# riveSunder/therldaisyworld

Hardware: AMD Instinct MI355X
Metric: cell-updates/sec (grid x batch), fused stencil+growth step (higher is better)
Workload: dtype f32

## Files before the change

therldaisyworld_amd/csrc/dw_api.hip:

```cpp
#include <hip/hip_runtime.h>

#include <cmath>
#include <cstdarg>
#include <cstdio>
#include <cstdlib>
#include <cstring>
#include <memory>
#include <new>
#include <type_traits>
#include <vector>

#include "../../include/daisyworld_hip.h"
#include "dw_kernels.hpp"
#include "dw_host_util.hpp"

using namespace dw;

static thread_local char g_err[512] = "";

static int fail(int code, const char* fmt, ...) {
    va_list ap;
    va_start(ap, fmt);
    vsnprintf(g_err, sizeof(g_err), fmt, ap);
    va_end(ap);
    return code;
}

#define HIPCHK(expr)                                                                           \
    do {                                                                                       \
        hipError_t e_ = (expr);                                                                \
        if (e_ != hipSuccess)                                                                  \
            return fail(e_ == hipErrorOutOfMemory ? DW_ENOMEM : DW_EHIP, "%s failed: %s (%s:%d)", \
                        #expr, hipGetErrorString(e_), __FILE__, __LINE__);                      \
    } while (0)

#define NEED(cond, code, ...)                      \
    do {                                           \
        if (!(cond)) return fail(code, __VA_ARGS__); \
    } while (0)

enum UnqKind { UNQ_F64 = 1, UNQ_F32 = 2 };
enum UnqOwner { OWN_NONE = 0, OWN_CUR = 1, OWN_PREV = 2 };

struct Switches {
    bool no_sym = false, no_pack = false, no_fuse = false, no_ring = false, no_episode_kernel = false,
         no_episode_wave = false, no_agent_fuse = false, no_agent_preapply = false, first_f64 = false,
         first_generic = false, force_rescan = false, test_hooks = false;
    int pack_min_strips = -1, strip_rows = 0, tile_rpt = 0, queue_cap = -1, mismatch_cap = -1;
    double first_slack = -1.0;
    char kernel[16] = {0};
    char text[256] = {0};
};
static const char* test_hook(const char* name) {
    return std::getenv("DW_TEST_HOOKS") ? std::getenv(name) : nullptr;
}
static Switches read_switches() {
    Switches w;
    auto note = [&](const char* name, const char* val) {
        const size_t n = std::strlen(w.text);
        snprintf(w.text + n, sizeof(w.text) - n, "%s%s%s%s", n ? " " : "", name, val ? "=" : "", val ? val : "");
    };
    auto flag = [&](const char* name, bool& dst) { if (std::getenv(name)) { dst = true; note(name, nullptr); } };
    auto num = [&](const char* name, int& dst, bool test) {
        if (const char* e = test ? test_hook(name) : std::getenv(name)) { dst = std::atoi(e); note(name, e); }
    };
    w.test_hooks = std::getenv("DW_TEST_HOOKS") != nullptr;
    flag("DW_NO_SYM", w.no_sym); flag("DW_NO_PACK", w.no_pack); flag("DW_NO_FUSE", w.no_fuse); flag("DW_NO_RING", w.no_ring);
    flag("DW_NO_EPISODE_KERNEL", w.no_episode_kernel); flag("DW_NO_EPISODE_WAVE", w.no_episode_wave);
    flag("DW_NO_AGENT_FUSE", w.no_agent_fuse); flag("DW_NO_AGENT_PREAPPLY", w.no_agent_preapply);
    flag("DW_FIRST_STEP_F64", w.first_f64); flag("DW_FIRST_GENERIC", w.first_generic);
    num("DW_PACK_MIN_STRIPS", w.pack_min_strips, false); num("DW_STRIP_ROWS", w.strip_rows, false);
    num("DW_TILE_RPT", w.tile_rpt, false);
    num("DW_TEST_QUEUE_CAP", w.queue_cap, true); num("DW_TEST_MISMATCH_CAP", w.mismatch_cap, true);
    if (test_hook("DW_TEST_FORCE_RESCAN")) { w.force_rescan = true; note("DW_TEST_FORCE_RESCAN", nullptr); }
    if (const char* e = test_hook("DW_TEST_FIRST_SLACK")) { w.first_slack = std::atof(e); note("DW_TEST_FIRST_SLACK", e); }
    if (const char* e = std::getenv("DW_KERNEL")) { snprintf(w.kernel, sizeof(w.kernel), "%s", e); note("DW_KERNEL", e); }
    return w;
}

enum StepKind { STEP_GENERIC, STEP_TILED, STEP_STREAM };
struct StepPlan {
    StepKind kind = STEP_GENERIC;
    int halo = 0;
    bool packed = false;
    bool allow_fuse = false;
    int fused_mode = kFusedOvl;
    bool sym_albedo = false;
    int tcq = 0, rpt = 0;
    Geom geom{};
    size_t tile_lds = 0;
    StripGeom sgeom{};
    FusedGeom fgeom{};
    int first_prec = 2;
    bool first_stream = false;
    FirstGeom first_geom{};
    bool need_fixq = false;
};

static thread_local int t_fail_in = 0;
struct DeviceMem {
    static int alloc(void** p, size_t n) {
        if (t_fail_in > 0 && --t_fail_in == 0) return hipErrorOutOfMemory;
        return hipMalloc(p, n);
    }
    static int release(void* p) { return hipFree(p); }
};
struct PinnedMem {
    static int alloc(void** p, size_t n) { return hipHostMalloc(p, n, hipHostMallocDefault); }
    static int release(void* p) { return hipHostFree(p); }
};
template <class T> using DevBuf = Buf<T, DeviceMem>;
template <class T> using PinnedBuf = Buf<T, PinnedMem>;

struct dw_handle {
    dw_params prm;
    hipStream_t stream = nullptr;
    bool own_stream = false;
    size_t cells = 0;
    DevBuf<plane_t> L16[2];
    DevBuf<plane_t> D16[2];
    int cur = 0;
    DevBuf<double> L64;
    DevBuf<double> D64;
    DevBuf<float> U32L;
    DevBuf<float> U32D;
    UnqKind unq_kind = UNQ_F64;
    UnqOwner unq = OWN_NONE;
    bool have_state = false;
    bool stepped = false;
    double L_last = 0.0;
    DevBuf<int> idx;
    DevBuf<double> st;
    DevBuf<int> action;
    DevBuf<int> action_tmp;
    bool have_agents = false;
    DevBuf<StatsDev> stats2[2];
    size_t stats_bytes = 0;
    int sp = 0;
    DevBuf<uint4> fixq;
    unsigned int qcap = 0;
    DevBuf<int> redo_tiles;
    Switches sw{};
    StepPlan plan{};
    DevBuf<int> done_at;
    DevBuf<int> agents_done_at;
// ... 315 lines not shown
static int halo_form(int W) { return W < 256 ? 3 : (W == 256 ? 0 : (W % 256 == 0 ? 1 : 2)); }

static int strip_rows(long groups, int H, long target) {
    int sr = 64;
    while (sr > 8 && groups * ((H + sr - 1) / sr) < target) sr >>= 1;
    return H < sr ? H : sr;
}

static StepPlan plan_steps(const dw_params& p, const Switches& sw) {
    StepPlan s;
    s.sym_albedo = (p.albedo_dark - p.albedo_bare) == -(p.albedo_light - p.albedo_bare) && !sw.no_sym;
    s.halo = halo_form(p.width);
    const int lpw = p.width / 4, wpr = lpw ? 64 / lpw : 0;
    const bool pack_shape = p.width >= 8 && p.width < 256 && wpr >= 1 && wpr * lpw * 10 >= 64 * 7 && !sw.no_pack;
    const long pack_strips = pack_shape ? (long)((p.batch + wpr - 1) / wpr) * ((p.height + 63) / 64) : 0;
    const bool packable = pack_shape && pack_strips >= (sw.pack_min_strips >= 0 ? sw.pack_min_strips : 512);
    const bool quads = p.precision != DW_PRECISION_F64 && p.width % 4 == 0;
    if (quads && (p.width >= 256 || packable) && std::strcmp(sw.kernel, "tiled") != 0) {
        s.kind = STEP_STREAM;
        s.packed = p.width < 256;
        StripGeom& g = s.sgeom;
        g.B = p.batch; g.H = p.height; g.W = p.width;
        g.ncs = (p.width + 255) / 256;
        g.lpw = s.packed ? lpw : 64;
        g.wpr = s.packed ? wpr : 1;
        const long groups = s.packed ? (p.batch + wpr - 1) / wpr : p.batch;
        g.SR = sw.strip_rows >= 1 ? (p.height < sw.strip_rows ? p.height : sw.strip_rows)
                                  : strip_rows(groups * g.ncs, p.height, 2048);
        g.nrs = (p.height + g.SR - 1) / g.SR;
        g.nstrips = (int)(groups * g.nrs * g.ncs);
        g.nwg = (g.nstrips + 3) / 4;
        g.chunk = (g.nwg + 7) / 8;
        g.qcap = kWaveQueueCap;
        int mcap = kMismatchCap;
        if (sw.queue_cap >= 0 && sw.queue_cap < kWaveQueueCap) g.qcap = sw.queue_cap;
        if (sw.mismatch_cap >= 0 && sw.mismatch_cap < kMismatchCap) mcap = sw.mismatch_cap;
        g.force_rescan = sw.force_rescan ? 1 : 0;
        s.allow_fuse = !sw.no_fuse;
        const bool ring = p.width == 1024 && !sw.no_ring;
        s.fused_mode = p.width <= 256 ? kFusedRot : (ring ? kFusedRing : kFusedOvl);
        FusedGeom& f = s.fgeom;
        f.B = p.batch; f.H = p.height; f.W = p.width;
        f.SR = g.SR;
        f.nrs = g.nrs;
        f.lpw = g.lpw; f.wpr = g.wpr;
        f.cols_per_strip = p.width <= 256 ? 256 : (ring ? 1024 : 248);
        f.ncs = s.packed ? 1 : (p.width + f.cols_per_strip - 1) / f.cols_per_strip;
        f.nstrips = (int)(groups * f.nrs * f.ncs);
        f.nwg = ring ? f.nstrips : (f.nstrips + 3) / 4;
        f.chunk = (f.nwg + 7) / 8;
        f.qcap = g.qcap;
        f.mcap = mcap;
        f.sure_need = 9 * p.n_agents + 9 * mcap + 1;
    } else if (quads && p.width >= 64) {
        s.kind = STEP_TILED;
        const int Wq = p.width / 4;
        if (Wq >= 64) {
            s.tcq = 64; s.rpt = 4;
            if (sw.tile_rpt == 2 || sw.tile_rpt == 4 || sw.tile_rpt == 8) s.rpt = sw.tile_rpt;
        }
        else if (Wq >= 32) { s.tcq = 32; s.rpt = 4; }
        else { s.tcq = 16; s.rpt = 2; }
        const int TR = (256 / s.tcq) * s.rpt;
        Geom& g = s.geom;
        g.B = p.batch; g.H = p.height; g.W = p.width; g.Wq = Wq;
        g.tiles_r = (p.height + TR - 1) / TR;
        g.tiles_c = (Wq + s.tcq - 1) / s.tcq;
        g.ntiles = p.batch * g.tiles_r * g.tiles_c;
        g.chunk = (g.ntiles + 7) / 8;
        g.qcap = kMaxFix;
        if (sw.queue_cap >= 0 && sw.queue_cap < kMaxFix) g.qcap = sw.queue_cap;
        s.tile_lds = (size_t)2 * (TR + 2) * (s.tcq + 2) * 4 * sizeof(float);
    }
    s.need_fixq = p.precision == DW_PRECISION_EXACT && s.kind == STEP_TILED;
    s.first_prec = p.precision == DW_PRECISION_FAST ? 1 : (p.precision == DW_PRECISION_EXACT && !sw.first_f64 ? 3 : 2);
    s.first_stream = (p.width % 256 == 0 || s.kind == STEP_STREAM) && s.first_prec != 2 && !sw.first_generic;
    if (s.first_stream) {
        FirstGeom& fg = s.first_geom;
        fg.B = p.batch; fg.H = p.height; fg.W = p.width;
        fg.lpw = s.packed ? lpw : 64;
        fg.wpr = s.packed ? wpr : 1;
        fg.ncs = s.packed ? 1 : (p.width + 255) / 256;
        const long groups = s.packed ? (p.batch + fg.wpr - 1) / fg.wpr : p.batch;
        fg.SR = strip_rows(groups * fg.ncs, p.height, 4096);
        fg.nrs = (p.height + fg.SR - 1) / fg.SR;
        fg.nstrips = (int)(groups * fg.nrs * fg.ncs);
    }
    return s;
}

static int ensure_fixq(dw_handle* h, const StepPlan& plan) {
    if (!plan.need_fixq) return DW_OK;
    const dw_params& p = h->prm;
    size_t per_q = (h->cells / 64 + kNumQueues - 1) / kNumQueues;
    if (per_q < 2048) per_q = 2048;
    per_q = (per_q + 255) / 256 * 256;
    const size_t max_tiles = (size_t)p.batch * ((p.height + 7) / 8) * ((p.width / 4 + 15) / 16);
    if (int rc = alloc_group(h, "the near-tie queues", {{h->fixq, sizeof(uint4) * 3 * per_q * kNumQueues},
                                                         {h->redo_tiles, sizeof(int) * max_tiles}}))
        return rc;
    h->qcap = (unsigned int)per_q;
    return DW_OK;
}

struct StepOut {
    plane_t* L; plane_t* D;
// ... 87 lines not shown
        auto tiled = [&](auto TCQ, auto RPT) {
            return with_bool(ex, [&](auto EX) { return launch_tiled<TCQ, RPT, EX>(h, iL, iD, o, fq); });
        };
        if (pl.tcq == 64) return with_int<8, 4, 2>(pl.rpt, [&](auto RPT) { return tiled(int_c<64>{}, RPT); });
        return pl.tcq == 32 ? tiled(int_c<32>{}, int_c<4>{}) : tiled(int_c<16>{}, int_c<2>{});
    }
    HIPCHK(hipGetLastError());
    return DW_OK;
}

static void step_done(dw_handle* h, double L, bool stepped) {
    h->cur = 1 - h->cur;
    h->sp = 1 - h->sp;
    h->unq = h->unq == OWN_CUR ? OWN_PREV : OWN_NONE;
    h->stepped = stepped;
    h->L_last = L;
    release_unquantised(h);
}

static int launch_forward(dw_handle* h, double L) {
    const dw_params& p = h->prm;
    NEED(h->have_state, DW_ESTATE, "no state uploaded (call dw_upload_state_* or dw_init_random)");
    const int out = 1 - h->cur;
    StatsDev* stats = h->stats2[1 - h->sp].get();
    const StepOut o{h->L16[out].get(), h->D16[out].get(), derive_f32(p, L), make_f64(p, L), stats, &stats[p.batch].sum_l,
                    reinterpret_cast<unsigned long long*>(h->stats2[h->sp].get()),
                    (int)(h->stats_bytes / sizeof(unsigned long long))};
#ifdef DW_TUNING
    if (const char* e = std::getenv("DW_ABLATE")) {
        if (std::strcmp(e, "copy") == 0) {
            const int in = h->cur;
            const size_t n4 = h->cells * sizeof(plane_t) / 16;
            hipLaunchKernelGGL(copy_planes, dim3((unsigned)((n4 + 255) / 256)), dim3(256), 0, h->stream,
                               reinterpret_cast<const float4*>(h->L16[in].get()), reinterpret_cast<const float4*>(h->D16[in].get()),
                               reinterpret_cast<float4*>(h->L16[out].get()), reinterpret_cast<float4*>(h->D16[out].get()), n4);
            HIPCHK(hipGetLastError());
            h->cur = out; h->sp = 1 - h->sp; h->stepped = true; h->L_last = L;
            return DW_OK;
        }
        const int v = std::strcmp(e, "nomath") == 0 ? 1 : 0;
        HIPCHK(hipMemcpyToSymbolAsync(HIP_SYMBOL(g_ablate), &v, sizeof(int), 0, hipMemcpyHostToDevice, h->stream));
    }
#endif
    if (int rc = h->unq == OWN_CUR ? launch_first_step(h, L, o) : launch_step(h, o)) return rc;
    step_done(h, L, true);
    return DW_OK;
}

template <class F>
static auto with_fused_layout(const StepPlan& pl, F&& f) {
    if (pl.packed) return f(int_c<kFusedRot>{}, std::true_type{});
    return with_int<kFusedRot, kFusedRing, kFusedOvl>(pl.fused_mode, [&](auto MODE) { return f(MODE, std::false_type{}); });
}

static int launch_forward_fused2(dw_handle* h, double L1, double L2, unsigned int* pstats = nullptr,
                                 float thr_hi = 0.f) {
    const dw_params& p = h->prm;
    const StepPlan& pl = h->plan;
    const int in = h->cur, out = 1 - h->cur;
    PhysF32 P1, P2;
    if (p.precision == DW_PRECISION_EXACT) derive_f32_pair(p, L1, L2, &P1, &P2);
    else { P1 = derive_f32(p, L1); P2 = derive_f32(p, L2); }
    unsigned long long* zero_me = reinterpret_cast<unsigned long long*>(h->stats2[h->sp].get());
    const int zero_n = (int)(h->stats_bytes / sizeof(unsigned long long));
    const FusedGeom& g = pl.fgeom;
    const dim3 grid((unsigned)g.chunk * 8u);
    if (p.precision == DW_PRECISION_EXACT) {
        const FusedExactArgs A{h->L16[in].get(), h->D16[in].get(), h->L16[out].get(), h->D16[out].get(), g, P1, lum_part(P2), zero_me, zero_n,
                               pstats, thr_hi, make_f64(p, L1), L1, L2};
        with_bool(pstats != nullptr, [&](auto STATS) {
            with_fused_layout(pl, [&](auto MODE, auto PACK) {
                with_bool(pl.sym_albedo, [&](auto SYM) {
                    hipLaunchKernelGGL((step_stream_fused2_exact<MODE, PACK, STATS, SYM>), grid, dim3(256), 0, h->stream, A);
                });
            });
        });
    } else {
        with_bool(pstats != nullptr, [&](auto STATS) {
            with_fused_layout(pl, [&](auto MODE, auto PACK) {
                hipLaunchKernelGGL((step_stream_fused2<MODE, PACK, STATS>), grid, dim3(256), 0, h->stream, h->L16[in].get(),
                                   h->D16[in].get(), h->L16[out].get(), h->D16[out].get(), g, P1, P2, zero_me, zero_n, pstats,
                                   thr_hi);
            });
        });
    }
    HIPCHK(hipGetLastError());
    step_done(h, L2, false);
    return DW_OK;
}

static int launch_agents(dw_handle* h, const int* d_action, int act_b, int act_n, bool standalone = false,
                         double* d_reward = nullptr, unsigned char* d_done = nullptr, unsigned char* d_ok = nullptr) {
    const dw_params& p = h->prm;
    if (p.n_agents == 0) return DW_OK;
    NEED(h->have_state, DW_ESTATE, "no state uploaded");
    NEED(h->have_agents, DW_ESTATE, "no agents uploaded (call dw_upload_agents or dw_init_random)");
    NEED(p.collision_mode == 0 || standalone, DW_EINVAL,
         "collision_mode=1: call dw_update_agents, apply the collision pass (it consumes the caller's RNG) to the "
         "downloaded agent states, upload them, then dw_step without actions");
    const int blocks = (p.batch + 63) / 64;
    with_planes(h, h->unq == OWN_CUR, h->cur, [&](auto* L, auto* D) {
        using T = elem_t<decltype(L)>;
        hipLaunchKernelGGL(agents_update<T>, dim3(blocks), dim3(64), 0, h->stream, L, D, h->idx.get(), h->st.get(), d_action,
                           act_b, act_n, p.batch, p.n_agents, p.height, p.width, p.agent_gamma,
                           p.collision_mode == 0 ? 1 : 0, d_reward, d_done, d_ok);
    });
    HIPCHK(hipGetLastError());
    return DW_OK;
}

static int stage_host_actions(dw_handle* h, const int32_t* action, int b, int n) {
    const dw_params& p = h->prm;
    NEED(b >= 0 && n >= 0 && b <= p.batch && n <= p.n_agents, DW_EINVAL,
         "action block %dx%d exceeds (B,N)=(%d,%d)", b, n, p.batch, p.n_agents);
    if ((size_t)b * n)
        HIPCHK(hipMemcpyAsync(h->action_tmp.get(), action, sizeof(int) * (size_t)b * n, hipMemcpyHostToDevice,
                              h->stream));
    return DW_OK;
}

extern "C" {

const char* dw_last_error(void) { return g_err; }
int dw_abi_version(void) { return DW_ABI_VERSION; }

int dw_pinned_alloc(size_t bytes, void** out) {
    NEED(out && bytes > 0, DW_EINVAL, "null argument");
    int ndev = 0;
    NEED(hipGetDeviceCount(&ndev) == hipSuccess && ndev > 0, DW_ENODEVICE, "no HIP device");
    HIPCHK(hipHostMalloc(out, bytes, hipHostMallocDefault));
    return DW_OK;
}
int dw_pinned_free(void* p) {
    if (p) HIPCHK(hipHostFree(p));
    return DW_OK;
}
// ... 1280 lines not shown
}

int dw_sync(dw_handle* h) {
    NEED(h, DW_EINVAL, "null handle");
    HIPCHK(hipSetDevice(h->prm.device));
    HIPCHK(hipStreamSynchronize(h->stream));
    return DW_OK;
}

int dw_timer_start(dw_handle* h) {
    NEED(h, DW_EINVAL, "null handle");
    HIPCHK(hipSetDevice(h->prm.device));
    HIPCHK(hipEventRecord(h->ev0, h->stream));
    return DW_OK;
}

int dw_timer_stop(dw_handle* h, float* elapsed_ms) {
    NEED(h && elapsed_ms, DW_EINVAL, "null argument");
    HIPCHK(hipSetDevice(h->prm.device));
    HIPCHK(hipEventRecord(h->ev1, h->stream));
    HIPCHK(hipEventSynchronize(h->ev1));
    HIPCHK(hipEventElapsedTime(elapsed_ms, h->ev0, h->ev1));
    return DW_OK;
}

int dw_device_planes(dw_handle* h, int which, void** light, void** dark) {
    NEED(h && light && dark, DW_EINVAL, "null argument");
    NEED(which == DW_STATE_CURRENT || which == DW_STATE_PREVIOUS, DW_EINVAL, "bad state selector");
    const int buf = which == DW_STATE_CURRENT ? h->cur : 1 - h->cur;
    NEED(which != DW_STATE_CURRENT || cur_quantised(h), DW_ESTATE,
         "the current state is an un-quantised upload: it has no binary16 planes before the first step");
    *light = h->L16[buf].get();
    *dark = h->D16[buf].get();
    return DW_OK;
}

int dw_kernel_info(dw_handle* h, char* buf, size_t buflen) {
    NEED(h && buf && buflen, DW_EINVAL, "null argument");
    const dw_params& p = h->prm;
    const StepPlan& pl = h->plan;
    const char* prec = p.precision == DW_PRECISION_EXACT ? "exact" : (p.precision == DW_PRECISION_FAST ? "fast" : "f64");
    static const char* const halo_name[] = {"rotate", "dpp-old", "general", "packed"};
    if (pl.kind == STEP_STREAM) {
        const StripGeom& g = pl.sgeom;
        snprintf(buf, buflen,
                 "step_stream_%s<halo=%s> wave-strip=%dx256 cells, register window + DPP neighbours, %d-row blocks in "
                 "flight%s, %d strips, grid=%d x 256 threads (4 strips each), XCD-chunked",
                 prec, halo_name[pl.halo], g.SR,
                 p.precision == DW_PRECISION_EXACT ? DW_STREAM_RB_EXACT : DW_STREAM_RB_FAST,
                 p.precision == DW_PRECISION_EXACT ? ", in-wave float64 fix-up from an LDS queue" : "", g.nstrips,
                 g.chunk * 8);
        if (pl.allow_fuse) {
            const size_t n = std::strlen(buf);
            snprintf(buf + n, buflen - n, "; dw_step_n fuses step pairs (step_stream_fused2%s)",
                     p.precision == DW_PRECISION_EXACT ? "_exact" : "");
        }
    } else if (pl.kind == STEP_TILED) {
        const int TR = (256 / pl.tcq) * pl.rpt;
        snprintf(buf, buflen,
                 "step_tiled<TCQ=%d,RPT=%d,%s> tile=%dx%d cells, %zu B LDS/workgroup, %d tiles, grid=%d x 256 threads, "
                 "XCD-chunked",
                 pl.tcq, pl.rpt, prec, TR, pl.tcq * 4, pl.tile_lds, pl.geom.ntiles, pl.geom.chunk * 8);
    } else {
        snprintf(buf, buflen, "step_generic<%s> one thread per cell, grid=(%d,%d) x 256 threads", prec,
                 (p.height * p.width + 255) / 256, p.batch);
    }
    if (h->sw.text[0]) {
        const size_t n = std::strlen(buf);
        snprintf(buf + n, buflen - n, "; switches[%s]", h->sw.text);
    }
    return DW_OK;
}

int dw_audit_tie_bound(dw_handle* h, double L, double out[4]) {
    NEED(h && out, DW_EINVAL, "null argument");
    const dw_params& p = h->prm;
    HIPCHK(hipSetDevice(p.device));
    NEED(h->have_state && cur_quantised(h), DW_ESTATE, "the audit needs a quantised current state");
    const StepPlan& pl = h->plan;
    int rc = ensure_scratch(h, 4 * sizeof(unsigned long long));
    if (rc) return rc;
    unsigned long long* d = reinterpret_cast<unsigned long long*>(h->scratch.get());
    HIPCHK(hipMemsetAsync(d, 0, 4 * sizeof(unsigned long long), h->stream));
    const dim3 g((unsigned)((p.height * p.width + 255) / 256), (unsigned)p.batch);
    hipLaunchKernelGGL(tie_audit, g, dim3(256), 0, h->stream, h->L16[h->cur].get(), h->D16[h->cur].get(), p.height, p.width,
                       derive_f32(p, L), make_f64(p, L), d, pl.sym_albedo && pl.kind == STEP_STREAM ? 1 : 0);
    HIPCHK(hipGetLastError());
    unsigned long long r[4];
    HIPCHK(hipMemcpyAsync(r, d, sizeof(r), hipMemcpyDeviceToHost, h->stream));
    HIPCHK(hipStreamSynchronize(h->stream));
    std::memcpy(&out[0], &r[0], sizeof(double));
    std::memcpy(&out[1], &r[1], sizeof(double));
    out[2] = (double)r[2];
    out[3] = (double)r[3];
    return DW_OK;
}

int dw_last_fixup_count(dw_handle* h, uint64_t* count) {
    NEED(h && count, DW_EINVAL, "null argument");
    HIPCHK(hipSetDevice(h->prm.device));
    std::vector<StatsDev> st((size_t)h->prm.batch + 1);
    HIPCHK(hipMemcpyAsync(st.data(), h->stats2[h->sp].get(), sizeof(StatsDev) * st.size(), hipMemcpyDeviceToHost, h->stream));
    HIPCHK(hipStreamSynchronize(h->stream));
    unsigned long long v = st[h->prm.batch].sum_l;
    for (int b = 0; b < h->prm.batch; ++b) v += st[b].reserved;
    *count = v;
    return DW_OK;
}
// ... 3 lines not shown
```

therldaisyworld_amd/csrc/dw_step_fused.hpp:

```cpp
#pragma once
#include <type_traits>
#include "dw_step_stream.hpp"

namespace dw {

struct FusedGeom {
    int B, H, W;
    int SR;
    int ncs, nrs;
    int nstrips, nwg, chunk;
    int cols_per_strip;
    int qcap, mcap;
    int lpw, wpr;
    int sure_need;
};

template <typename TI>
__device__ inline unsigned int exact1_word(const TI* __restrict__ pL, const TI* __restrict__ pD, int H, int W,
                                           int r, int c, const PhysF64& Pa) {
    const int rr = wrap_near2(r, H), cc = wrap_near2(c, W);
    const int ru = rr == 0 ? H - 1 : rr - 1, rd = rr == H - 1 ? 0 : rr + 1;
    const int cl = cc == 0 ? W - 1 : cc - 1, cr = cc == W - 1 ? 0 : cc + 1;
    const int rows[3] = {ru, rr, rd}, cols[3] = {cl, cc, cr};
    unsigned int w1[9];
#pragma unroll
    for (int x = 0; x < 3; ++x)
#pragma unroll
        for (int y = 0; y < 3; ++y) {
            const size_t o = (size_t)rows[x] * W + cols[y];
            w1[x * 3 + y] = (unsigned)(float)pL[o] | ((unsigned)(float)pD[o] << 16);
        }
    const NewCoverF64 s1 = cell_f64_lean(Pa, w1);
    return (unsigned)dw_round3_k(s1.nl) | ((unsigned)dw_round3_k(s1.nd) << 16);
}

template <typename TI>
__device__ inline void exact2_cell(const TI* __restrict__ pL, const TI* __restrict__ pD, int H, int W, int r,
                                   int c, const PhysF64& Pa, const PhysF64& Pb, float& kl, float& kd) {
    unsigned int w2[9];
#pragma unroll
    for (int a = 0; a < 3; ++a)
#pragma unroll
        for (int e = 0; e < 3; ++e) {
            int rr = r + a - 1, cc = c + e - 1;
            rr = rr < 0 ? rr + H : (rr >= H ? rr - H : rr);
            cc = cc < 0 ? cc + W : (cc >= W ? cc - W : cc);
            const int ru = rr == 0 ? H - 1 : rr - 1, rd = rr == H - 1 ? 0 : rr + 1;
            const int cl = cc == 0 ? W - 1 : cc - 1, cr = cc == W - 1 ? 0 : cc + 1;
            const int rows[3] = {ru, rr, rd}, cols[3] = {cl, cc, cr};
            unsigned int w1[9];
#pragma unroll
            for (int x = 0; x < 3; ++x)
#pragma unroll
                for (int y = 0; y < 3; ++y) {
                    const size_t o = (size_t)rows[x] * W + cols[y];
                    w1[x * 3 + y] = (unsigned)(float)pL[o] | ((unsigned)(float)pD[o] << 16);
                }
            const NewCoverF64 s1 = cell_f64_lean(Pa, w1);
            w2[a * 3 + e] = (unsigned)dw_round3_k(s1.nl) | ((unsigned)dw_round3_k(s1.nd) << 16);
        }
    const NewCoverF64 s2 = cell_f64_lean(Pb, w2);
    kl = (float)dw_round3_k(s2.nl);
    kd = (float)dw_round3_k(s2.nd);
}

constexpr int kMismatchCap = 64;

enum { kFusedOvl = 0, kFusedRot = 1, kFusedRing = 2 };
template <int MODE, bool EXACT, bool PACK = false, bool STATS = false, bool SYM = false, typename TI = plane_t,
          typename TO = plane_t>
__device__ __forceinline__ void fused2_body(const TI* __restrict__ inL, const TI* __restrict__ inD,
                                            TO* __restrict__ outL, TO* __restrict__ outD, const FusedGeom& G,
                                            const PhysF32& P1_, const PhysF32& P2_, const PhysF64& P64,
                                            const double& La, const double& Lb,
                                            unsigned long long* __restrict__ zero_me, int zero_n,
                                            unsigned int* __restrict__ pstats = nullptr, float thr_hi = 0.f) {
#ifndef DW_FUSED_LAG
#define DW_FUSED_LAG 1
#endif
    constexpr bool LAG = DW_FUSED_LAG != 0;
    constexpr bool ROT = MODE == kFusedRot, RING = MODE == kFusedRing;
    static_assert(!RING || (LAG && !PACK), "the ring exchange is written for the lagged loop of un-packed worlds");
    __shared__ float s_edge[RING ? 2 * 4 * 8 : 1];
    __shared__ uint4 s_queue[EXACT ? 4 * kWaveQueueCap * 3 : 1];
    __shared__ unsigned int s_mm[EXACT ? 4 * kMismatchCap : 1];
    const int bid = blockIdx.x;
    const int wg = (bid & 7) * G.chunk + (bid >> 3);
    if (wg >= G.nwg) return;
    const int tid = threadIdx.x, wv = tid >> 6, lane = tid & 63;
    if (wg == 0)
        for (int i = tid; i < zero_n; i += 256) zero_me[i] = 0ull;
    const int s = RING ? wg : __builtin_amdgcn_readfirstlane(wg * 4 + wv);
    if (!RING && s >= G.nstrips) return;
    uint4* q = s_queue + (EXACT ? wv * kWaveQueueCap * 3 : 0);
    unsigned int* mm = s_mm + (EXACT ? wv * kMismatchCap : 0);
    const int spw = G.nrs * G.ncs;
    const int b = s / spw;
    const int sw = s - b * spw;
    const int rs = sw / G.ncs, cs = sw - rs * G.ncs;
    const int r0 = rs * G.SR;
    const int nr = min(G.SR, G.H - r0);
    const int pw = PACK ? lane / G.lpw : 0, pj = PACK ? lane - pw * G.lpw : 0;
    const int lsrc = PACK ? (pj == 0 ? lane + G.lpw - 1 : lane - 1) : 0;
    const int rsrc = PACK ? (pj == G.lpw - 1 ? lane - (G.lpw - 1) : lane + 1) : 0;
    auto world_off = [&](int lc) -> size_t {
        return (size_t)(PACK ? min(b * G.wpr + min((lc >> 2) / G.lpw, G.wpr - 1), G.B - 1) : b) * G.H * G.W;
    };
    const size_t woff = world_off(4 * lane);
    const int c00 = ROT ? 0 : (RING ? 256 * __builtin_amdgcn_readfirstlane(wv) : cs * 248 - 4);
    int col = PACK ? 4 * pj : c00 + 4 * lane;
    col = col < 0 ? col + G.W : col;
    col = col >= G.W ? col - G.W : col;
    const bool writes = PACK ? (pw < G.wpr && b * G.wpr + pw < G.B)
                             : ((ROT || RING) ? true : (lane >= 1 && lane <= 62 && cs * 248 + 4 * (lane - 1) < G.W));
    bool need1[4] = {true, true, true, true};
    if (PACK) { need1[0] = need1[1] = need1[2] = need1[3] = writes; }
    if (EXACT && !ROT && !RING) {
        const bool wl = __builtin_amdgcn_update_dpp(0, writes ? 1 : 0, kDppWaveShr1, 0xf, 0xf, false) != 0;
        const bool wr = __builtin_amdgcn_update_dpp(0, writes ? 1 : 0, kDppWaveShl1, 0xf, 0xf, false) != 0;
        need1[0] = writes || wl;
        need1[1] = writes;
        need1[2] = writes;
        need1[3] = writes || wr;
    }
    constexpr bool LANE_BOOLS = PACK || (STATS && MODE == kFusedOvl);
    using TieT = std::conditional_t<LANE_BOOLS, bool, unsigned long long>;
    TieT need1m[4], writes_m;
    if constexpr (LANE_BOOLS) {
        for (int i = 0; i < 4; ++i) need1m[i] = need1[i];
        writes_m = writes;
    } else {
        for (int i = 0; i < 4; ++i) need1m[i] = lane_mask(need1[i]);
        writes_m = lane_mask(writes);
    }
    const TI* pL = inL + woff;
    const TI* pD = inD + woff;

    struct RawIn { dw_f16x4 l, d; };
    auto load_raw = [&](int rr) -> RawIn {
        rr = min(rr, r0 + nr + 1);
        rr = rr < 0 ? rr + G.H : rr;
        rr = rr >= G.H ? rr - G.H : rr;
        RawIn w;
        w.l = stream_load4_raw(pL + (size_t)rr * G.W + col);
        w.d = stream_load4_raw(pD + (size_t)rr * G.W + col);
        return w;
    };
    auto pin_edge_sums = [&](Row4& L, Row4& D) {
        asm volatile("" : "+v"(L.h2[0]), "+v"(L.h2[3]), "+v"(D.h2[0]), "+v"(D.h2[3]));
    };
    auto nbrs = [&](const float4& v, float& a, float& c) {
        if (PACK) { a = __shfl(v.w, lsrc, 64); c = __shfl(v.x, rsrc, 64); }
        else if (ROT) { a = dpp_mov_nb<kDppWaveRor1>(v.w); c = dpp_mov_nb<kDppWaveRol1>(v.x); }
        else { a = dpp_mov_nb<kDppWaveShr1>(v.w); c = dpp_mov_nb<kDppWaveShl1>(v.x); }
    };
    auto to_rows4 = [&](const float4& l, const float4& d, Row4& L, Row4& D) {
        float a, c;
        nbrs(l, a, c);
        L = make_row(l, a, c);
        nbrs(d, a, c);
        D = make_row(d, a, c);
    };
    int ring_par = 0;
    auto rows_ring = [&](const float4* v, Row4* const* out, auto NC) {
        constexpr int n = decltype(NC)::value;
        float* mine = s_edge + (ring_par * 4 + wv) * 8;
        if (lane == 63) {
#pragma unroll
            for (int i = 0; i < n; ++i) mine[i] = v[i].w;
        }
        if (lane == 0) {
#pragma unroll
            for (int i = 0; i < n; ++i) mine[4 + i] = v[i].x;
        }
        __syncthreads();
        const float* lw = s_edge + (ring_par * 4 + ((wv + 3) & 3)) * 8;
        const float* rw = s_edge + (ring_par * 4 + ((wv + 1) & 3)) * 8 + 4;
#pragma unroll
        for (int i = 0; i < n; ++i) {
            const float a = dpp_mov<kDppWaveShr1>(lw[i], v[i].w);
            const float c = dpp_mov<kDppWaveShl1>(rw[i], v[i].x);
            *out[i] = make_row(v[i], a, c);
        }
        ring_par ^= 1;
    };
    unsigned int nq = 0;
#ifndef DW_PIN_CONSTS
#define DW_PIN_CONSTS -1
#endif
    PhysF32 P1 = P1_, P2 = P2_;
    constexpr int PIN = DW_PIN_CONSTS < 0 ? (MODE == kFusedOvl ? 14 : (MODE == kFusedRing ? 8 : 0)) : DW_PIN_CONSTS;
    if constexpr (EXACT && PIN != 0 && !STATS && !PACK) {
        if constexpr ((PIN & 1) != 0) asm volatile("" : "+v"(P1.c0l), "+v"(P2.c0l));
        if constexpr ((PIN & 2) != 0) { asm volatile("" : "+v"(P1.pck)); P2.pck = P1.pck; }
        if constexpr ((PIN & 4) != 0) { asm volatile("" : "+v"(P1.eKb)); P2.eKb = P1.eKb; }
        if constexpr ((PIN & 8) != 0) { asm volatile("" : "+v"(P1.gt)); P2.gt = P1.gt; }
    }
    constexpr bool CHEAP = STATS && !PACK;
    static_assert(LAG || !CHEAP, "the dependent-order loop (DW_FUSED_LAG=0, experiments) keeps the per-lane statistics");
    float st_m1 = 0.f, st_x1 = 0.f;
    unsigned int st_c2 = 0, st_nmm = 0, st_c2w = 0;
    bool st_sure1 = false;
    const unsigned long long writes_mask = CHEAP ? lane_mask(writes) : 0ull;
    const float thr_c2 = EXACT ? thr_hi + 1.0f : thr_hi;
    auto row_map = [&](const PhysF32& P, const Row4& upL, const Row4& miL, const Row4& dnL, const Row4& upD,
                       const Row4& miD, const Row4& dnD, float4& nl, float4& nd, int kind, int lrow,
                       const TieT* use, float* sure_max = nullptr) {
        float ol[4], od[4];
        TieT tie[4];
        cells4<EXACT, SYM, TieT>(P, upL, miL, dnL, upD, miD, dnD, ol, od, tie);
        if (EXACT) {
#pragma unroll
            for (int i = 0; i < 4; ++i) tie[i] = tie[i] & use[i];
        }
        if (STATS && sure_max) {
// ... 108 lines not shown
                if (e < nq) {
                    const uint4 e0 = q[e * 3], e1 = q[e * 3 + 1], e2 = q[e * 3 + 2];
                    const unsigned int w[9] = {unpack_ld(e0.z), unpack_ld(e0.w), unpack_ld(e1.x),
                                               unpack_ld(e1.y), unpack_ld(e1.z), unpack_ld(e1.w),
                                               unpack_ld(e2.x), unpack_ld(e2.y), unpack_ld(e2.z)};
                    Pe.L = e0.x == 1u ? la : lb;
                    const NewCoverF64 o = cell_f64_lean(Pe, w);
                    const unsigned int kl = (unsigned)dw_round3_k(o.nl), kd = (unsigned)dw_round3_k(o.nd);
                    where = e0.y;
                    if (e0.x == 1u) {
                        mism = (kl | (kd << 16)) != unpack_ld(e2.w);
                        if (STATS && is_output((int)(where >> 16), (int)(where & 0xffffu))) {
                            const unsigned int mx = kl > kd ? kl : kd;
                            if (PACK) atomicMax(&pstats[2 * world_of((int)(where & 0xffffu))], mx);
                            else st_x1 = fmaxf(st_x1, (float)mx);
                        }
                    } else {
                        int gr, gc;
                        size_t wo;
                        locate((int)(where >> 16), (int)(where & 0xffffu), wo, gr, gc);
                        const size_t off = wo + (size_t)gr * G.W + gc;
                        outL[off] = (TO)(float)kl;
                        outD[off] = (TO)(float)kd;
                    }
                }
                const unsigned long long mask = lane_mask(mism);
                if (mism) {
                    const unsigned int slot = nmm + __builtin_amdgcn_mbcnt_hi((unsigned)(mask >> 32),
                                                                             __builtin_amdgcn_mbcnt_lo((unsigned)mask, 0u));
                    if (slot < (unsigned)G.mcap) mm[slot] = where;
                }
                nmm += (unsigned)__popcll(mask);
            }
            __builtin_amdgcn_fence(__ATOMIC_RELEASE, "wavefront");
            __builtin_amdgcn_wave_barrier();
        }
        nq = 0;
    };

    Row4 IL[3], ID[3], SL[3], SD[3];
    {
        const RawIn p0 = load_raw(r0 - 2), p1 = load_raw(r0 - 1), p2 = load_raw(r0);
        if constexpr (RING) {
            const float4 va[4] = {widen4(p0.l), widen4(p0.d), widen4(p1.l), widen4(p1.d)};
            const float4 vb[2] = {widen4(p2.l), widen4(p2.d)};
            Row4* const oa[4] = {&IL[0], &ID[0], &IL[1], &ID[1]};
            Row4* const ob[2] = {&IL[2], &ID[2]};
            rows_ring(va, oa, std::integral_constant<int, 4>{});
            rows_ring(vb, ob, std::integral_constant<int, 2>{});
        } else {
            to_rows4(widen4(p0.l), widen4(p0.d), IL[0], ID[0]);
            to_rows4(widen4(p1.l), widen4(p1.d), IL[1], ID[1]);
            to_rows4(widen4(p2.l), widen4(p2.d), IL[2], ID[2]);
        }
    }
    using U0 = std::integral_constant<int, 0>;
    using U1 = std::integral_constant<int, 1>;
    using U2 = std::integral_constant<int, 2>;
    if constexpr (LAG) {
        auto iter = [&](auto U, auto D1, auto D2, int j, auto ST) {
            constexpr int u = decltype(U)::value;
            constexpr bool do1 = decltype(D1)::value, do2 = decltype(D2)::value;
            constexpr bool st_on = STATS && decltype(ST)::value;
            RawIn nx;
            if (do1) nx = load_raw(r0 + j);
            __builtin_amdgcn_sched_barrier(0);
            float l1[4], d1[4], l2[4], d2[4];
            TieT tie1[4], tie2[4];
            float sm1 = 0.f, sm2 = 0.f;
            if (do2)
                row_cells(P2, SL[u], SL[(u + 1) % 3], SL[(u + 2) % 3], SD[u], SD[(u + 1) % 3], SD[(u + 2) % 3], l2, d2, tie2,
                          use2, st_on ? &sm2 : nullptr);
            if (do1)
                row_cells(P1, IL[(u + 2) % 3], IL[u], IL[(u + 1) % 3], ID[(u + 2) % 3], ID[u], ID[(u + 1) % 3], l1, d1, tie1,
                          need1m, st_on ? &sm1 : nullptr);
            if (do2) {
                row_queue(SL[u], SL[(u + 1) % 3], SL[(u + 2) % 3], SD[u], SD[(u + 1) % 3], SD[(u + 2) % 3], l2, d2, tie2, 2,
                          j - 2);
                if (st_on) stats_step2(sm2);
                if (writes) {
                    const size_t off = woff + (size_t)(r0 + j - 4) * G.W + col;
                    stream_store4(outL + off, make_float4(l2[0], l2[1], l2[2], l2[3]));
                    stream_store4(outD + off, make_float4(d2[0], d2[1], d2[2], d2[3]));
                }
            }
            if (do1) {
                row_queue(IL[(u + 2) % 3], IL[u], IL[(u + 1) % 3], ID[(u + 2) % 3], ID[u], ID[(u + 1) % 3], l1, d1, tie1, 1, j);
                if (st_on) stats_step1(sm1, l1, d1, tie1, j >= 2 && j <= nr + 1);
                if constexpr (RING) {
                    const float4 v[4] = {make_float4(l1[0], l1[1], l1[2], l1[3]), make_float4(d1[0], d1[1], d1[2], d1[3]),
                                         widen4(nx.l), widen4(nx.d)};
                    Row4* const o[4] = {&SL[u], &SD[u], &IL[(u + 2) % 3], &ID[(u + 2) % 3]};
                    rows_ring(v, o, std::integral_constant<int, 4>{});
                } else {
                    to_rows4(make_float4(l1[0], l1[1], l1[2], l1[3]), make_float4(d1[0], d1[1], d1[2], d1[3]), SL[u], SD[u]);
                    __builtin_amdgcn_sched_barrier(0);
                    to_rows4(widen4(nx.l), widen4(nx.d), IL[(u + 2) % 3], ID[(u + 2) % 3]);
                    if (!PACK) pin_edge_sums(IL[(u + 2) % 3], ID[(u + 2) % 3]);
                }
            }
        };
        using Yes = std::true_type;
        using No = std::false_type;
        iter(U1{}, Yes{}, No{}, 1, Yes{});
        iter(U2{}, Yes{}, No{}, 2, Yes{});
        iter(U0{}, Yes{}, No{}, 3, Yes{});
        const int jend = nr + 2;
        int j = 4;
        for (; j + 2 <= jend; j += 3) {
            iter(U1{}, Yes{}, Yes{}, j, Yes{});
            iter(U2{}, Yes{}, Yes{}, j + 1, Yes{});
            iter(U0{}, Yes{}, Yes{}, j + 2, Yes{});
            if (EXACT && !STATS && __builtin_expect(nq >= (unsigned)flush_at, 0)) sweep_queue();
            if (CHEAP && st_sure1 && st_c2w >= (unsigned int)G.sure_need) { j += 3; break; }
        }
        if constexpr (CHEAP) {
            for (; j + 2 <= jend; j += 3) {
                iter(U1{}, Yes{}, Yes{}, j, No{});
                iter(U2{}, Yes{}, Yes{}, j + 1, No{});
                iter(U0{}, Yes{}, Yes{}, j + 2, No{});
            }
        }
        if (j <= jend) { iter(U1{}, Yes{}, Yes{}, j, Yes{}); ++j; }
        if (j <= jend) { iter(U2{}, Yes{}, Yes{}, j, Yes{}); ++j; }
        if (j % 3 == 1) iter(U1{}, No{}, Yes{}, j, Yes{});
        else if (j % 3 == 2) iter(U2{}, No{}, Yes{}, j, Yes{});
        else iter(U0{}, No{}, Yes{}, j, Yes{});
    } else {
        auto iter = [&](auto U, int j) {
            constexpr int u = decltype(U)::value;
            const RawIn nx = load_raw(r0 + j);
            __builtin_amdgcn_sched_barrier(0);
            float4 l1, d1;
            float sm = 0.f;
            row_map(P1, IL[(u + 2) % 3], IL[u], IL[(u + 1) % 3], ID[(u + 2) % 3], ID[u], ID[(u + 1) % 3], l1, d1, 1, j, need1m,
                    STATS ? &sm : nullptr);
            if (STATS && writes && j >= 2 && j <= nr + 1) st_m1 = fmaxf(st_m1, sm);
            to_rows4(l1, d1, SL[u], SD[u]);
            if (j >= 3) {
                float4 l2, d2;
                row_map(P2, SL[(u + 1) % 3], SL[(u + 2) % 3], SL[u], SD[(u + 1) % 3], SD[(u + 2) % 3], SD[u], l2, d2, 2, j - 1,
                        use2, STATS ? &sm : nullptr);
                if (STATS && writes && sm > thr_hi) st_c2 += 1u;
                if (writes) {
                    const size_t off = woff + (size_t)(r0 + j - 3) * G.W + col;
                    stream_store4(outL + off, l2);
                    stream_store4(outD + off, d2);
                }
            }
            __builtin_amdgcn_sched_barrier(0);
// ... 184 lines not shown
```

Before: 768.6 billion.

## Add column-pass fused layout with full 256-column strips for fast-precision step pairs

For fast-precision fused step pairs on widths divisible by 256 (other than 1024), this adds a new kFusedCol layout. Each wave owns a full 256-column strip with no overlap. The halo columns on either side are precomputed once per strip into LDS (raw values plus first-step results) and folded into the edge lanes' neighbour sums with masked FMAs. This removes the redundant overlapped-column work of the 248-column layout, where only lanes 1..62 wrote output. It also lets strips grow taller (SR doubled up to 256 while enough strips remain), cutting halo row overhead. The cost is an upfront column pass, extra LDS, and more per-row work on edge lanes.

```diff
diff --git a/therldaisyworld_amd/csrc/dw_api.hip b/therldaisyworld_amd/csrc/dw_api.hip
--- a/therldaisyworld_amd/csrc/dw_api.hip
+++ b/therldaisyworld_amd/csrc/dw_api.hip
@@ -43,7 +43,7 @@
 enum UnqOwner { OWN_NONE = 0, OWN_CUR = 1, OWN_PREV = 2 };
 
 struct Switches {
-    bool no_sym = false, no_pack = false, no_fuse = false, no_ring = false, no_episode_kernel = false,
+    bool no_sym = false, no_pack = false, no_fuse = false, no_ring = false, no_fused_col = false, no_episode_kernel = false,
          no_episode_wave = false, no_agent_fuse = false, no_agent_preapply = false, first_f64 = false,
          first_generic = false, force_rescan = false, test_hooks = false;
     int pack_min_strips = -1, strip_rows = 0, tile_rpt = 0, queue_cap = -1, mismatch_cap = -1;
@@ -66,6 +66,7 @@
     };
     w.test_hooks = std::getenv("DW_TEST_HOOKS") != nullptr;
     flag("DW_NO_SYM", w.no_sym); flag("DW_NO_PACK", w.no_pack); flag("DW_NO_FUSE", w.no_fuse); flag("DW_NO_RING", w.no_ring);
+    flag("DW_NO_FUSED_COL", w.no_fused_col);
     flag("DW_NO_EPISODE_KERNEL", w.no_episode_kernel); flag("DW_NO_EPISODE_WAVE", w.no_episode_wave);
     flag("DW_NO_AGENT_FUSE", w.no_agent_fuse); flag("DW_NO_AGENT_PREAPPLY", w.no_agent_preapply);
     flag("DW_FIRST_STEP_F64", w.first_f64); flag("DW_FIRST_GENERIC", w.first_generic);
@@ -91,6 +92,8 @@
     size_t tile_lds = 0;
     StripGeom sgeom{};
     FusedGeom fgeom{};
+    int fast_mode = kFusedOvl;
+    FusedGeom fast_geom{};
     int first_prec = 2;
     bool first_stream = false;
     FirstGeom first_geom{};
@@ -512,6 +515,25 @@
         f.qcap = g.qcap;
         f.mcap = mcap;
         f.sure_need = 9 * p.n_agents + 9 * mcap + 1;
+        s.fast_mode = s.fused_mode;
+        s.fast_geom = f;
+        if (p.precision == DW_PRECISION_FAST && s.fused_mode == kFusedOvl) {
+            FusedGeom& c = s.fast_geom;
+            if (p.width % 256 == 0 && p.width != 1024 && !sw.no_fused_col) {
+                s.fast_mode = kFusedCol;
+                c.cols_per_strip = 256;
+                c.ncs = p.width / 256;
+            }
+            const long slots = 256L * 16;
+            if (sw.strip_rows < 1)
+                while (c.SR >= 64 && c.SR < kColMaxSR && groups * c.ncs * ((p.height + 2 * c.SR - 1) / (2 * c.SR)) >= 8 * slots)
+                    c.SR *= 2;
+            if (c.SR > kColMaxSR) c.SR = kColMaxSR;
+            c.nrs = (p.height + c.SR - 1) / c.SR;
+            c.nstrips = (int)(groups * c.nrs * c.ncs);
+            c.nwg = (c.nstrips + 3) / 4;
+            c.chunk = (c.nwg + 7) / 8;
+        }
     } else if (quads && p.width >= 64) {
         s.kind = STEP_TILED;
         const int Wq = p.width / 4;
@@ -705,6 +727,11 @@
     if (pl.packed) return f(int_c<kFusedRot>{}, std::true_type{});
     return with_int<kFusedRot, kFusedRing, kFusedOvl>(pl.fused_mode, [&](auto MODE) { return f(MODE, std::false_type{}); });
 }
+template <class F>
+static auto with_fast_layout(const StepPlan& pl, F&& f) {
+    if (pl.packed) return f(int_c<kFusedRot>{}, std::true_type{});
+    return with_int<kFusedRot, kFusedRing, kFusedCol, kFusedOvl>(pl.fast_mode, [&](auto MODE) { return f(MODE, std::false_type{}); });
+}
 
 static int launch_forward_fused2(dw_handle* h, double L1, double L2, unsigned int* pstats = nullptr,
                                  float thr_hi = 0.f) {
@@ -716,7 +743,8 @@
     else { P1 = derive_f32(p, L1); P2 = derive_f32(p, L2); }
     unsigned long long* zero_me = reinterpret_cast<unsigned long long*>(h->stats2[h->sp].get());
     const int zero_n = (int)(h->stats_bytes / sizeof(unsigned long long));
-    const FusedGeom& g = pl.fgeom;
+    const bool plain_fast = p.precision != DW_PRECISION_EXACT && pstats == nullptr;
+    const FusedGeom& g = plain_fast ? pl.fast_geom : pl.fgeom;
     const dim3 grid((unsigned)g.chunk * 8u);
     if (p.precision == DW_PRECISION_EXACT) {
         const FusedExactArgs A{h->L16[in].get(), h->D16[in].get(), h->L16[out].get(), h->D16[out].get(), g, P1, lum_part(P2), zero_me, zero_n,
@@ -728,13 +756,17 @@
                 });
             });
         });
+    } else if (plain_fast) {
+        with_fast_layout(pl, [&](auto MODE, auto PACK) {
+            hipLaunchKernelGGL((step_stream_fused2<MODE, PACK, false>), grid, dim3(256), 0, h->stream, h->L16[in].get(),
+                               h->D16[in].get(), h->L16[out].get(), h->D16[out].get(), g, P1, P2, zero_me, zero_n, pstats,
+                               thr_hi);
+        });
     } else {
-        with_bool(pstats != nullptr, [&](auto STATS) {
-            with_fused_layout(pl, [&](auto MODE, auto PACK) {
-                hipLaunchKernelGGL((step_stream_fused2<MODE, PACK, STATS>), grid, dim3(256), 0, h->stream, h->L16[in].get(),
-                                   h->D16[in].get(), h->L16[out].get(), h->D16[out].get(), g, P1, P2, zero_me, zero_n, pstats,
-                                   thr_hi);
-            });
+        with_fused_layout(pl, [&](auto MODE, auto PACK) {
+            hipLaunchKernelGGL((step_stream_fused2<MODE, PACK, true>), grid, dim3(256), 0, h->stream, h->L16[in].get(),
+                               h->D16[in].get(), h->L16[out].get(), h->D16[out].get(), g, P1, P2, zero_me, zero_n, pstats,
+                               thr_hi);
         });
     }
     HIPCHK(hipGetLastError());
@@ -2121,8 +2153,18 @@
                  g.chunk * 8);
         if (pl.allow_fuse) {
             const size_t n = std::strlen(buf);
-            snprintf(buf + n, buflen - n, "; dw_step_n fuses step pairs (step_stream_fused2%s)",
-                     p.precision == DW_PRECISION_EXACT ? "_exact" : "");
+            static const char* const layout_name[] = {"overlapped 248-column strips", "rotating 256-column strips",
+                                                      "ring of four 256-column strips", "256-column strips + column pass"};
+            const bool fast = p.precision == DW_PRECISION_FAST;
+            const int mode = pl.packed ? kFusedRot : (fast ? pl.fast_mode : pl.fused_mode);
+            snprintf(buf + n, buflen - n, "; dw_step_n fuses step pairs (step_stream_fused2%s, %s%s of %d rows)",
+                     p.precision == DW_PRECISION_EXACT ? "_exact" : "", pl.packed ? "packed worlds in " : "", layout_name[mode],
+                     fast ? pl.fast_geom.SR : pl.fgeom.SR);
+            if (fast && p.n_agents > 0 && (pl.fast_mode != pl.fused_mode || pl.fast_geom.SR != pl.fgeom.SR)) {
+                const size_t m = std::strlen(buf);
+                snprintf(buf + m, buflen - m, "; pairs with agents in between: %s of %d rows", layout_name[pl.fused_mode],
+                         pl.fgeom.SR);
+            }
         }
     } else if (pl.kind == STEP_TILED) {
         const int TR = (256 / pl.tcq) * pl.rpt;
diff --git a/therldaisyworld_amd/csrc/dw_step_fused.hpp b/therldaisyworld_amd/csrc/dw_step_fused.hpp
--- a/therldaisyworld_amd/csrc/dw_step_fused.hpp
+++ b/therldaisyworld_amd/csrc/dw_step_fused.hpp
@@ -66,7 +66,8 @@
 
 constexpr int kMismatchCap = 64;
 
-enum { kFusedOvl = 0, kFusedRot = 1, kFusedRing = 2 };
+enum { kFusedOvl = 0, kFusedRot = 1, kFusedRing = 2, kFusedCol = 3 };
+constexpr int kColMaxSR = 256, kColRows = kColMaxSR + 5;
 template <int MODE, bool EXACT, bool PACK = false, bool STATS = false, bool SYM = false, typename TI = plane_t,
           typename TO = plane_t>
 __device__ __forceinline__ void fused2_body(const TI* __restrict__ inL, const TI* __restrict__ inD,
@@ -79,8 +80,10 @@
 #define DW_FUSED_LAG 1
 #endif
     constexpr bool LAG = DW_FUSED_LAG != 0;
-    constexpr bool ROT = MODE == kFusedRot, RING = MODE == kFusedRing;
+    constexpr bool ROT = MODE == kFusedRot, RING = MODE == kFusedRing, COL = MODE == kFusedCol;
     static_assert(!RING || (LAG && !PACK), "the ring exchange is written for the lagged loop of un-packed worlds");
+    static_assert(!COL || (LAG && !EXACT && !PACK && !STATS), "the column pass serves the plain float32-only pairs");
+    __shared__ float s_col[COL ? 4 * kColRows * 8 : 1];
     __shared__ float s_edge[RING ? 2 * 4 * 8 : 1];
     __shared__ uint4 s_queue[EXACT ? 4 * kWaveQueueCap * 3 : 1];
     __shared__ unsigned int s_mm[EXACT ? 4 * kMismatchCap : 1];
@@ -100,6 +103,9 @@
     const int rs = sw / G.ncs, cs = sw - rs * G.ncs;
     const int r0 = rs * G.SR;
     const int nr = min(G.SR, G.H - r0);
+#ifndef DW_COL_SPLIT
+#define DW_COL_SPLIT 1
+#endif
     const int pw = PACK ? lane / G.lpw : 0, pj = PACK ? lane - pw * G.lpw : 0;
     const int lsrc = PACK ? (pj == 0 ? lane + G.lpw - 1 : lane - 1) : 0;
     const int rsrc = PACK ? (pj == G.lpw - 1 ? lane - (G.lpw - 1) : lane + 1) : 0;
@@ -107,12 +113,12 @@
         return (size_t)(PACK ? min(b * G.wpr + min((lc >> 2) / G.lpw, G.wpr - 1), G.B - 1) : b) * G.H * G.W;
     };
     const size_t woff = world_off(4 * lane);
-    const int c00 = ROT ? 0 : (RING ? 256 * __builtin_amdgcn_readfirstlane(wv) : cs * 248 - 4);
+    const int c00 = ROT ? 0 : (RING ? 256 * __builtin_amdgcn_readfirstlane(wv) : (COL ? cs * 256 : cs * 248 - 4));
     int col = PACK ? 4 * pj : c00 + 4 * lane;
     col = col < 0 ? col + G.W : col;
     col = col >= G.W ? col - G.W : col;
     const bool writes = PACK ? (pw < G.wpr && b * G.wpr + pw < G.B)
-                             : ((ROT || RING) ? true : (lane >= 1 && lane <= 62 && cs * 248 + 4 * (lane - 1) < G.W));
+                             : ((ROT || RING) ? true : COL ? (DW_COL_SPLIT ? c00 + 4 * lane < G.W : true) : (lane >= 1 && lane <= 62 && cs * 248 + 4 * (lane - 1) < G.W));
     bool need1[4] = {true, true, true, true};
     if (PACK) { need1[0] = need1[1] = need1[2] = need1[3] = writes; }
     if (EXACT && !ROT && !RING) {
@@ -161,6 +167,51 @@
         nbrs(d, a, c);
         D = make_row(d, a, c);
     };
+    float col_m0 = lane == 0 ? 1.0f : 0.0f, col_m63 = lane == 63 ? 1.0f : 0.0f;
+    if constexpr (COL) asm volatile("" : "+v"(col_m0), "+v"(col_m63));
+    auto add_side = [&](float hl, float hd, Row4& L, Row4& D) {
+        L.h2[0] = __builtin_fmaf(hl, col_m0, L.h2[0]);
+        L.h2[3] = __builtin_fmaf(hl, col_m63, L.h2[3]);
+        D.h2[0] = __builtin_fmaf(hd, col_m0, D.h2[0]);
+        D.h2[3] = __builtin_fmaf(hd, col_m63, D.h2[3]);
+    };
+    const float* col_e = s_col + (COL ? (wv * kColRows * 2 + (lane >> 5)) * 4 : 0);
+    auto col_entry = [&](int k) -> float4 { return *reinterpret_cast<const float4*>(col_e + k * 8); };
+    if constexpr (COL) {
+        float* cw = s_col + wv * kColRows * 8;
+        const int hc[2] = {c00 == 0 ? G.W - 1 : c00 - 1, c00 + 256 == G.W ? 0 : c00 + 256};
+        for (int base = 0; base < nr + 3; base += 62) {
+            const int k = base + lane;
+            int rr = min(r0 - 2 + k, r0 + nr + 1);
+            rr = rr < 0 ? rr + G.H : rr;
+            rr = rr >= G.H ? rr - G.H : rr;
+            const TI* rl = pL + (size_t)rr * G.W;
+            const TI* rd = pD + (size_t)rr * G.W;
+#pragma unroll
+            for (int side = 0; side < 2; ++side) {
+                const int c = hc[side], cl = c == 0 ? G.W - 1 : c - 1, cr = c == G.W - 1 ? 0 : c + 1;
+                const float xl = (float)rl[c], xd = (float)rd[c];
+                const float hl = (float)rl[cl] + (float)rl[cr], hd = (float)rd[cl] + (float)rd[cr];
+                const float El = hl + (dpp_mov_nb<kDppWaveShr1>(xl) + dpp_mov_nb<kDppWaveShl1>(xl));
+                const float Cl = dpp_mov_nb<kDppWaveShr1>(hl) + dpp_mov_nb<kDppWaveShl1>(hl);
+                const float Ed = hd + (dpp_mov_nb<kDppWaveShr1>(xd) + dpp_mov_nb<kDppWaveShl1>(xd));
+                const float Cd = dpp_mov_nb<kDppWaveShr1>(hd) + dpp_mov_nb<kDppWaveShl1>(hd);
+                const GrowthT<float> g = growth_t<kFastSplit, float>(P1_, xl, xd, El, Cl, Ed, Cd);
+                const float vl = finish_fast_t<float>(xl, g.dKl, g.fl), vd = finish_fast_t<float>(xd, g.dKd, g.fd);
+                if (k <= nr + 4) {
+                    cw[k * 8 + side * 4 + 0] = xl;
+                    cw[k * 8 + side * 4 + 1] = xd;
+                }
+                if (lane >= 1 && lane <= 62 && k <= nr + 2) {
+                    cw[(k + 2) * 8 + side * 4 + 2] = vl;
+                    cw[(k + 2) * 8 + side * 4 + 3] = vd;
+                }
+            }
+        }
+        __builtin_amdgcn_fence(__ATOMIC_RELEASE, "wavefront");
+        __builtin_amdgcn_wave_barrier();
+        __builtin_amdgcn_fence(__ATOMIC_ACQUIRE, "wavefront");
+    }
     int ring_par = 0;
     auto rows_ring = [&](const float4* v, Row4* const* out, auto NC) {
         constexpr int n = decltype(NC)::value;
@@ -375,6 +426,13 @@
             to_rows4(widen4(p0.l), widen4(p0.d), IL[0], ID[0]);
             to_rows4(widen4(p1.l), widen4(p1.d), IL[1], ID[1]);
             to_rows4(widen4(p2.l), widen4(p2.d), IL[2], ID[2]);
+            if constexpr (COL) {
+#pragma unroll
+                for (int k = 0; k < 3; ++k) {
+                    const float4 e = col_entry(k);
+                    add_side(e.x, e.y, IL[k], ID[k]);
+                }
+            }
         }
     }
     using U0 = std::integral_constant<int, 0>;
@@ -386,6 +444,7 @@
             constexpr bool do1 = decltype(D1)::value, do2 = decltype(D2)::value;
             constexpr bool st_on = STATS && decltype(ST)::value;
             RawIn nx;
+            float4 ce;
             if (do1) nx = load_raw(r0 + j);
             __builtin_amdgcn_sched_barrier(0);
             float l1[4], d1[4], l2[4], d2[4];
@@ -397,6 +456,7 @@
             if (do1)
                 row_cells(P1, IL[(u + 2) % 3], IL[u], IL[(u + 1) % 3], ID[(u + 2) % 3], ID[u], ID[(u + 1) % 3], l1, d1, tie1,
                           need1m, st_on ? &sm1 : nullptr);
+            if (COL && do1) ce = col_entry(j + 2);
             if (do2) {
                 row_queue(SL[u], SL[(u + 1) % 3], SL[(u + 2) % 3], SD[u], SD[(u + 1) % 3], SD[(u + 2) % 3], l2, d2, tie2, 2,
                           j - 2);
@@ -417,8 +477,10 @@
                     rows_ring(v, o, std::integral_constant<int, 4>{});
                 } else {
                     to_rows4(make_float4(l1[0], l1[1], l1[2], l1[3]), make_float4(d1[0], d1[1], d1[2], d1[3]), SL[u], SD[u]);
+                    if constexpr (COL) add_side(ce.z, ce.w, SL[u], SD[u]);
                     __builtin_amdgcn_sched_barrier(0);
                     to_rows4(widen4(nx.l), widen4(nx.d), IL[(u + 2) % 3], ID[(u + 2) % 3]);
+                    if constexpr (COL) add_side(ce.x, ce.y, IL[(u + 2) % 3], ID[(u + 2) % 3]);
                     if (!PACK) pin_edge_sums(IL[(u + 2) % 3], ID[(u + 2) % 3]);
                 }
             }
```

Result: slower. 756.1 billion (median of 2 runs) (-1.6%).
